# FengHZ/SHOT-VAE

Hardware: AMD Instinct MI355X
Metric: images/sec/step WRN-28-2 SHOT-VAE CIFAR-10 bs512 (higher is better)
Workload: dtype bf16; 1 GPU; SHOT-VAE train step (4 fwd + 2 bwd + SGD) wideresnet-28-2 K=10 ldc=128, B_l=B_u=512 per GPU, synthetic 3x32x32 in HBM, random init; global_batch=1024, parallelism=dp1, schedule=grouped (forwards (1)-(4) as one batched launch sequence, 4 BatchNorm groups), launch=eager, weight gradients on a side stream, collective=none

## Files before the change

include/shotvae_hip.h:

```cpp
#ifndef SHOTVAE_HIP_H
#define SHOTVAE_HIP_H

#include <stdint.h>

#ifdef __cplusplus
extern "C" {
#endif

#define SV_ABI_VERSION 8

enum { SV_F32 = 0, SV_BF16 = 1 };
typedef double sv_acc_t;
enum { SV_OK = 0, SV_E_ARG = -1, SV_E_SHAPE = -2, SV_E_HIP = -3 };
enum { SV_MAX_TAPS = 16, SV_MAX_PHASES = 4 };

typedef struct {
    int32_t ooy, oox;
    int32_t ntap;
    int8_t dy[SV_MAX_TAPS];
    int8_t dx[SV_MAX_TAPS];
    int8_t torig[SV_MAX_TAPS];
    int64_t w_off;
} sv_phase;

// ... 276 lines not shown
int sv_prof_enable(int on);
int sv_prof_tag(int tag);
int sv_prof_nested_tag(int tag);
int sv_prof_nested_tag_kind(int kind, int tag);
int sv_prof_collect(int max_tags, double* ms, int* count);

int sv_debug_wgrad_tile_program(int halo_vectors, int* items, int* waits);

int sv_debug_conv_chunk_program(int* items, int* waits);

enum { SV_OPT_DISABLE_MASK = 0, SV_OPT_WIDE_MIN_BLOCKS = 1, SV_OPT_HALO_ALL = 2, SV_OPT_PERSISTENT_BLOCKS = 3,
       SV_OPT_DETERMINISTIC = 4, SV_OPT_ENABLE_MASK = 5 };
enum { SV_K_CONV3X3 = 1, SV_K_CONV3X3P = 2, SV_K_CONV3X3M = 4, SV_K_CONV3X3W = 8, SV_K_CONV3X3X = 16,
       SV_K_WGRAD3X3 = 32, SV_K_WGRAD3X3W = 64, SV_K_IGEMM_KV2 = 128, SV_K_HALO = 256, SV_K_HALOP = 512, SV_K_HWGRAD = 1024, SV_K_IGEMM_BIG = 2048, SV_K_WGRAD_WIDE = 4096, SV_K_IGEMM_ALIGNED = 8192, SV_K_IGEMM_DMA = 16384, SV_K_WGRAD_INCR = 32768, SV_K_WGRAD3X3M = 65536, SV_K_TCONVR = 131072, SV_K_TCONVR_EX = 262144, SV_K_SCONV = 524288, SV_K_PCONV = 8388608, SV_K_THCONV = 16777216, SV_K_THWGRAD = 67108864, SV_K_S2WGRAD = 134217728,
       SV_K_MAP4 = 268435456,
       SV_K_MAP4_CONV = 536870912   };
int sv_set_option(int key, int value);
int sv_get_option(int key);

int sv_stream_fork(void* from, void* to, int light);
int sv_stream_flag_next(void* stream, uint32_t** flag, uint32_t* value);
int sv_stream_wait_flag(void* stream, const uint32_t* flag, uint32_t value);
int sv_flag_timeouts(void);
int sv_flag_timeouts_reset(void);

int sv_version(void);
const char* sv_last_error(void);

#ifdef __cplusplus
}
#endif
// ... 2 lines not shown
```

shot_vae_amd/_lib.py:

```python
import ctypes as C
import os
import subprocess

HERE = os.path.dirname(os.path.abspath(__file__))
LIB_PATH = os.environ.get("SV_LIB_PATH") or os.path.join(HERE, "libshotvae_hip.so")
CSRC = os.path.join(HERE, "csrc")

SV_F32, SV_BF16 = 0, 1
ABI_VERSION = 8
MAX_TAPS, MAX_PHASES = 16, 4


class SvPhase(C.Structure):
    _fields_ = [("ooy", C.c_int32), ("oox", C.c_int32), ("ntap", C.c_int32),
                ("dy", C.c_int8 * MAX_TAPS), ("dx", C.c_int8 * MAX_TAPS), ("torig", C.c_int8 * MAX_TAPS),
                ("w_off", C.c_int64)]


class SvGeom(C.Structure):
    _fields_ = [("B", C.c_int32), ("Hin", C.c_int32), ("Win", C.c_int32), ("Cin", C.c_int32), ("ldx", C.c_int32),
                ("Hq", C.c_int32), ("Wq", C.c_int32), ("sy", C.c_int32), ("sx", C.c_int32),
                ("Hout", C.c_int32), ("Wout", C.c_int32), ("N", C.c_int32), ("ldo", C.c_int32),
                ("osy", C.c_int32), ("osx", C.c_int32), ("T_orig", C.c_int32), ("nphase", C.c_int32),
                ("phase", SvPhase * MAX_PHASES)]
# ... 151 lines not shown
    "sv_bn_bwd_apply_dropout": [I, I64, I, I, P, P, P, F, C.POINTER(SvBnBranch), I, P, P, I, C.POINTER(SvDropoutArgs), P],
    "sv_dropout_mask": [P, I, C.c_uint32, I64, I, I, P, P],
    "sv_stream_fork": [P, P, I],
    "sv_stream_flag_next": [P, P, P],
    "sv_stream_wait_flag": [P, P, C.c_uint32],
    "sv_flag_timeouts": [],
    "sv_flag_timeouts_reset": [],
    "sv_version": [],
}
OPT_DISABLE_MASK, OPT_WIDE_MIN_BLOCKS, OPT_HALO_ALL, OPT_PERSISTENT_BLOCKS, OPT_DETERMINISTIC, OPT_ENABLE_MASK = 0, 1, 2, 3, 4, 5
(K_CONV3X3, K_CONV3X3P, K_CONV3X3M, K_CONV3X3W, K_CONV3X3X, K_WGRAD3X3, K_WGRAD3X3W, K_IGEMM_KV2, K_HALO, K_HALOP, K_HWGRAD, K_IGEMM_BIG,
 K_WGRAD_WIDE, K_IGEMM_ALIGNED, K_IGEMM_DMA, K_WGRAD_INCR, K_WGRAD3X3M, K_TCONVR, K_TCONVR_EX, K_SCONV) = (1 << i for i in range(20))
K_PCONV, K_THCONV, K_THWGRAD, K_S2WGRAD = 1 << 23, 1 << 24, 1 << 26, 1 << 27
K_MAP4 = 1 << 28
K_MAP4_CONV = 1 << 29
EXPORTS = sorted(list(_PROTOS) + ["sv_last_error"])

_lib = None


class ShotVaeHipError(RuntimeError):
    pass


def build(verbose=False):
    r = subprocess.run(["make", "-C", CSRC, "-j4"], capture_output=True, text=True)
    if verbose or r.returncode != 0:
        print(r.stdout[-4000:])
        print(r.stderr[-4000:])
    if r.returncode != 0:
# ... 87 lines not shown
```

shot_vae_amd/csrc/bwd3x3f.hip:

```cpp
#include "common.h"
#include "epilogue.h"

int sv_bwd3x3_64(const sv_geom* g, const sv_bwd3x3_args* a, hipStream_t s);

namespace {

constexpr int LDF = 48;
constexpr int LDR = 40;
constexpr int CH = 32;
#ifndef SV_BWDF_WREGS
#define SV_BWDF_WREGS 2
#endif
#ifndef SV_BWDF_ABL
#define SV_BWDF_ABL 0
#endif

struct bwdf_params {
    const void* dy;
    const void* dy2;
    const void* dy3;
    void* dy_out;
    const float* dy_scale;
    const float* dy_scale2;
    const float* dy_shift;
// ... 18 lines not shown
    int fold_replicas;
};
struct bwdf_g { bwdf_params g[SV_MAX_GROUPS]; };

__device__ __forceinline__ bf16x8 ftr(const bf16* S, int pix_elem_q, int col0, int lane) {
    typedef __attribute__((address_space(3))) s16x4 lds_v4;
    const bf16* a0 = S + pix_elem_q + col0 + 4 * (lane & 3);
    const s16x4 lo = __builtin_amdgcn_ds_read_tr16_b64_v4i16((lds_v4*)(a0));
    const s16x4 hi = __builtin_amdgcn_ds_read_tr16_b64_v4i16((lds_v4*)(a0 + 4 * LDF));
    union { s16x4 s[2]; bf16x8 b; } u;
    u.s[0] = lo;
    u.s[1] = hi;
    return u.b;
}

template <int NS, int MODE>
struct bwdf_stage {
    bf16x8 gv[NS];
    bf16x8 yv[MODE >= 1 ? NS : 1];
    bf16x8 rv[MODE == 2 ? NS : 1];
    bf16x8 xv;
};

template <int WLOG, int MODE>
__global__ __launch_bounds__(512) void bwd3x3f_kernel(const sv_geom g, const bwdf_g PG) {
    const bwdf_params& p = PG.g[blockIdx.y];
    typedef bf16x8 V;
    typedef bf16x4 Q;
    constexpr int WREGS = WLOG == 5 ? SV_BWDF_WREGS : (MODE == 0 ? 1 : 0);
    constexpr int FRAGS = WLOG == 5 ? 1 : 2;
    constexpr bool GFIRST = MODE >= 1;
    constexpr int WLROWS = (2 - WREGS) * 16 * 9;
    constexpr int W = 1 << WLOG, TR = 128 / W, WP = W + 2;
    constexpr int HH = (TR < W) ? TR : W, SEG = TR / HH, LROWS = TR + SEG + 1, HP = LROWS * WP;
    constexpr int HV = LROWS * W * 4;
    static_assert(HV > 512 && HV <= 768, "slots: vectors 0..511 on the weight-gradient waves (two each), 512.. on the others (one each)");
    constexpr int SDY = HP * LDF, SAC = 128 * LDF, SXR = 128 * LDR, STG = SDY + SAC + SXR;
    static_assert((SDY * 2) % 16 == 0 && (SAC * 2) % 16 == 0 && (STG * 2) % 16 == 0, "16-byte aligned LDS images");

    extern __shared__ __attribute__((aligned(16))) char smem[];
    bf16* const st0 = reinterpret_cast<bf16*>(smem);
    double* const ssum = reinterpret_cast<double*>(st0 + 2 * STG);
    float* const cf = reinterpret_cast<float*>(ssum + 2 * CH);
    bf16* const wl = reinterpret_cast<bf16*>(cf + 8 * CH);

    const int tid = threadIdx.x, lane = tid & 63;
    const int wave = __builtin_amdgcn_readfirstlane(tid >> 6);
// ... 9 lines not shown
    const char* __restrict__ X = reinterpret_cast<const char*>(p.x);
    bf16* __restrict__ O = reinterpret_cast<bf16*>(p.out);
    float slope = p.x_slope;
    asm volatile("v_mov_b32 %0, %0" : "+v"(slope));

    if (MODE >= 1 && p.fold_bsums) {
        sv_bn_bwd_affine_block512<CH>(p.fold_bsums, p.fold_replicas, p.fold_inv_count, p.fold_gamma, p.fold_mean, p.fold_rstd,
                                      p.fold_dgamma, p.fold_dbeta, blockIdx.x == 0, reinterpret_cast<double*>(smem), cf);
    }
    if (tid < CH) {
        if (MODE >= 1 && !p.fold_bsums) {
            cf[tid] = p.dy_scale[tid];
            cf[CH + tid] = p.dy_scale2[tid];
            cf[2 * CH + tid] = p.dy_shift[tid];
        }
        cf[3 * CH + tid] = p.x_scale[tid];
        cf[4 * CH + tid] = p.x_shift[tid];
        cf[5 * CH + tid] = p.x_mean[tid];
        cf[6 * CH + tid] = p.x_rstd[tid];
    }
    if (tid < 2 * CH) ssum[tid] = 0.0;
    for (int idx = tid; idx < 2 * LROWS * 2 * 4; idx += 512) {
        const int vv = idx & 3, side = (idx >> 2) & 1, row = (idx >> 3) % LROWS, stg = (idx >> 3) / LROWS;
        bf16x8 z;
#pragma unroll
        for (int j = 0; j < 8; ++j) z[j] = (bf16)0.f;
        *reinterpret_cast<bf16x8*>(st0 + stg * STG + (row * WP + side * (WP - 1)) * LDF + 8 * vv) = z;
    }

    const int v = tid & 3;
    int hlds[2];
    uint32_t hoff[2];
#pragma unroll
    for (int i = 0; i < 2; ++i) {
        const int idx = wave >= 4 ? (tid - 256) + 256 * i : (i == 0 ? 512 + tid : HV);
        const int pix = min(idx, HV - 1) >> 2;
        const int lr = pix >> WLOG, xx = pix & (W - 1);
        const int seg = lr / (HH + 1), off = lr - seg * (HH + 1);
        int kind = 1, rel = lr - 1 - seg;
        if (off == 0) {
            if (SEG == 1) { kind = seg == 0 ? 2 : 3; rel = seg == 0 ? -1 : TR; }
            else kind = 0;
        }
        hoff[i] = (uint32_t)(((rel + 1) * W + xx) * CH + 8 * v) * 2u;
        hlds[i] = idx < HV ? (((lr * WP + xx + 1) * LDF + 8 * v) | kind) : -1;
    }
    const uint32_t hsafe = (uint32_t)(W * CH + 8 * v) * 2u;
    const int cp = tid >> 2;
    const uint32_t coff = (uint32_t)(cp * CH + 8 * v) * 2u;

    auto load_stage = [&](auto& S, int tile) __attribute__((always_inline)) {
        constexpr int NS = sizeof(S.gv) / sizeof(V);
        const int gr0 = tile * TR;
        const bool top_ok = (gr0 & (H - 1)) != 0, bot_ok = ((gr0 + TR) & (H - 1)) != 0;
        const int64_t hb = ((int64_t)gr0 - 1) * W * CH * 2;
#pragma unroll
        for (int i = 0; i < NS; ++i) {
            const int kind = hlds[i] & 3;
            const bool ok = hlds[i] >= 0 && (kind == 1 || (kind == 2 && top_ok) || (kind == 3 && bot_ok));
            const uint32_t o = ok ? hoff[i] : hsafe;
            S.gv[i] = *reinterpret_cast<const V*>(DY + hb + o);
            if constexpr (MODE >= 1) S.yv[i] = *reinterpret_cast<const V*>(DY2 + hb + o);
            if constexpr (MODE == 2) S.rv[i] = *reinterpret_cast<const V*>(DY3 + hb + o);
        }
        S.xv = *reinterpret_cast<const V*>(X + (int64_t)gr0 * W * CH * 2 + coff);
    };
    V zero;
#pragma unroll
    for (int j = 0; j < 8; ++j) zero[j] = (bf16)0.f;
    auto store_stage = [&](auto& S, int tile, int stage) __attribute__((always_inline)) {
        constexpr int NS = sizeof(S.gv) / sizeof(V);
        bf16* sb = st0 + stage * STG;
        const int gr0 = tile * TR;
        const bool top_ok = (gr0 & (H - 1)) != 0, bot_ok = ((gr0 + TR) & (H - 1)) != 0;
        const int64_t hb = ((int64_t)gr0 - 1) * W * CH * 2;
#pragma unroll
        for (int i = 0; i < NS; ++i) {
            const int kind = hlds[i] & 3;
            const bool ok = kind == 1 || (kind == 2 && top_ok) || (kind == 3 && bot_ok);
            V o = S.gv[i];
// ... 5 lines not shown
                    const f32x4 cc = *reinterpret_cast<const f32x4*>(cf + 2 * CH + 8 * v + 4 * h);
#pragma unroll
                    for (int j = 0; j < 4; ++j) {
                        float t = to_f(S.gv[i][4 * h + j]) * ca[j] + (to_f(S.yv[MODE >= 1 ? i : 0][4 * h + j]) * cb[j] + cc[j]);
                        if constexpr (MODE == 2) t += to_f(S.rv[MODE == 2 ? i : 0][4 * h + j]);
                        o[4 * h + j] = (bf16)t;
                    }
                }
                if constexpr (MODE == 2) {
                    if (hlds[i] >= 0 && kind == 1) *reinterpret_cast<V*>(DYO + hb + hoff[i]) = o;
                }
            }
            if (!ok) o = zero;
            if (hlds[i] >= 0) *reinterpret_cast<V*>(sb + (hlds[i] & ~7)) = o;
        }
        const f32x4 s0 = *reinterpret_cast<const f32x4*>(cf + 3 * CH + 8 * v), s1 = *reinterpret_cast<const f32x4*>(cf + 3 * CH + 8 * v + 4);
        const f32x4 t0 = *reinterpret_cast<const f32x4*>(cf + 4 * CH + 8 * v), t1 = *reinterpret_cast<const f32x4*>(cf + 4 * CH + 8 * v + 4);
        *reinterpret_cast<V*>(sb + SDY + cp * LDF + 8 * v) = bn_act8(S.xv, s0, s1, t0, t1, slope);
        *reinterpret_cast<V*>(sb + SDY + SAC + cp * LDR + 8 * v) = S.xv;
    };

    const int dwave = wave & 3;
    int hbase[2], prow[2], pcol[2];
#pragma unroll
    for (int ms = 0; ms < 2; ++ms) {
        const int pp = 32 * dwave + 16 * ms + fr;
        prow[ms] = pp >> WLOG;
        pcol[ms] = pp & (W - 1);
        hbase[ms] = ((prow[ms] + 1 + prow[ms] / HH) * WP + pcol[ms] + 1) * LDF + 8 * fq;
    }
    V wr[9][WREGS > 0 ? WREGS : 1];
    float s1[2][4], s2[2][4];
#pragma unroll
    for (int i = 0; i < 2; ++i)
#pragma unroll
        for (int r = 0; r < 4; ++r) s1[i][r] = s2[i][r] = 0.f;
    {
        const bf16* Wp = reinterpret_cast<const bf16*>(p.w) + P.w_off;
        if (wave < 4) {
#pragma unroll
            for (int t = 0; t < 9; ++t)
#pragma unroll
                for (int i = 0; i < WREGS; ++i) wr[t][i] = *reinterpret_cast<const V*>(Wp + ((16 * i + fr) * 9 + t) * CH + 8 * fq);
        }
        for (int idx = tid; idx < WLROWS * 4; idx += 512)
            *reinterpret_cast<V*>(wl + (idx >> 2) * LDF + 8 * (idx & 3)) =
                *reinterpret_cast<const V*>(Wp + (WREGS * 16 * 9 + (idx >> 2)) * CH + 8 * (idx & 3));
    }
    auto compute_d = [&](int tile, int stage) __attribute__((always_inline)) {
        const bf16* dyh = st0 + stage * STG;
        const bf16* xr = dyh + SDY + SAC;
        f32x4 acc[2][2];
#pragma unroll
        for (int i = 0; i < 2; ++i)
#pragma unroll
            for (int j = 0; j < 2; ++j) acc[i][j] = f32x4{0.f, 0.f, 0.f, 0.f};
#pragma unroll
        for (int t = 0; t < 9; ++t) {
            const int sh = ((1 - t / 3) * WP + (1 - t % 3)) * LDF;
            const V af0 = *reinterpret_cast<const V*>(dyh + hbase[0] + sh);
            const V af1 = *reinterpret_cast<const V*>(dyh + hbase[1] + sh);
#pragma unroll
            for (int i = 0; i < 2; ++i) {
                const V wf = i < WREGS ? wr[t][i < WREGS ? i : 0] : *reinterpret_cast<const V*>(wl + (((i - WREGS) * 16 + fr) * 9 + t) * LDF + 8 * fq);
                mma32(acc[i][0], wf, af0);
                mma32(acc[i][1], wf, af1);
            }
        }
        const int gr0 = tile * TR;
        if (SV_BWDF_ABL & 16) {
#pragma unroll
            for (int i = 0; i < 2; ++i)
#pragma unroll
                for (int ms = 0; ms < 2; ++ms) s1[i][ms] += acc[i][ms][0] + acc[i][ms][1] + acc[i][ms][2] + acc[i][ms][3];
            return;
        }
#pragma unroll
        for (int i = 0; i < 2; ++i) {
            const int c = 16 * i + 4 * fq;
            const f32x4 esc = *reinterpret_cast<const f32x4*>(cf + 3 * CH + c), esh = *reinterpret_cast<const f32x4*>(cf + 4 * CH + c);
            const f32x4 emu = *reinterpret_cast<const f32x4*>(cf + 5 * CH + c), ers = *reinterpret_cast<const f32x4*>(cf + 6 * CH + c);
#pragma unroll
            for (int ms = 0; ms < 2; ++ms) {
                const Q xq = *reinterpret_cast<const Q*>(xr + (32 * dwave + 16 * ms + fr) * LDR + c);
                f32x4 vv = acc[i][ms];
                Q o;
#pragma unroll
                for (int r = 0; r < 4; ++r) {
                    const float xf = to_f(xq[r]);
                    const float gv = vv[r] * act_grad(xf * esc[r] + esh[r], slope);
                    s1[i][r] += gv;
                    s2[i][r] += gv * ((xf - emu[r]) * ers[r]);
                    o[r] = (bf16)gv;
                }
                *reinterpret_cast<Q*>(O + ((int64_t)(gr0 + prow[ms]) * W + pcol[ms]) * CH + c) = o;
            }
        }
    };

    const int wi = (wave >> 1) & 1, wj = wave & 1;
    f32x4 dacc[9];
#pragma unroll
    for (int t = 0; t < 9; ++t) dacc[t] = f32x4{0.f, 0.f, 0.f, 0.f};
    auto compute_g = [&](int stage) __attribute__((always_inline)) {
        const bf16* dyh = st0 + stage * STG;
        const bf16* ac = dyh + SDY;
        auto frag_b = [&](int kc) __attribute__((always_inline)) {
            const int pq = 32 * kc + 8 * fq + (fr >> 2);
            return ftr(ac, pq * LDF, 16 * wj, lane);
        };
        auto frag_a = [&](int kc, int t) __attribute__((always_inline)) {
            const int pq = 32 * kc + 8 * fq + (fr >> 2);
            const int jrow = pq >> WLOG, xcol = pq & (W - 1);
            const int hb = ((jrow + 1 + jrow / HH) * WP + xcol + 1) * LDF;
            return ftr(dyh, hb + ((1 - t / 3) * WP + (1 - t % 3)) * LDF, 16 * wi, lane);
        };
        if constexpr (FRAGS == 1) {
#pragma unroll
            for (int kc = 0; kc < 4; ++kc) {
                const bf16x8 fb = frag_b(kc);
                bf16x8 fa[9];
#pragma unroll
                for (int t = 0; t < 9; ++t) fa[t] = frag_a(kc, t);
#pragma unroll
                for (int t = 0; t < 9; ++t) dacc[t] = __builtin_amdgcn_mfma_f32_16x16x32_bf16(fa[t], fb, dacc[t], 0, 0, 0);
            }
        } else {
#pragma unroll
            for (int kc = 0; kc < 4; ++kc) {
                const bf16x8 fb = frag_b(kc);
                bf16x8 fa[5];
#pragma unroll
                for (int t = 0; t < 5; ++t) fa[t] = frag_a(kc, t);
#pragma unroll
                for (int t = 0; t < 5; ++t) dacc[t] = __builtin_amdgcn_mfma_f32_16x16x32_bf16(fa[t], fb, dacc[t], 0, 0, 0);
#pragma unroll
                for (int t = 5; t < 9; ++t) fa[t - 5] = frag_a(kc, t);
#pragma unroll
                for (int t = 5; t < 9; ++t) dacc[t] = __builtin_amdgcn_mfma_f32_16x16x32_bf16(fa[t - 5], fb, dacc[t], 0, 0, 0);
            }
        }
    };

    auto tile_barrier = [&]() __attribute__((always_inline)) { asm volatile("s_waitcnt lgkmcnt(0)\n\ts_barrier" ::: "memory"); };
// ... 11 lines not shown
        load_stage(SB, min(t_begin + tstep, t_last));
        __syncthreads();
        store_stage(SA, t_begin, 0);
        load_stage(SA, min(t_begin + 2 * tstep, t_last));
        __syncthreads();
        int tile = t_begin;
        for (int k = 0; k + 1 < n_tiles; k += 2, tile += 2 * tstep) {
            iter(tile, 0, SB);
            iter(tile + tstep, 1, SA);
        }
        if (n_tiles & 1) {
            if (!(SV_BWDF_ABL & 2)) compute_d(tile, 0);
            tile_barrier();
        }
#pragma unroll
        for (int i = 0; i < 2; ++i)
#pragma unroll
            for (int r = 0; r < 4; ++r) {
                s1[i][r] = row16_sum(s1[i][r]);
                s2[i][r] = row16_sum(s2[i][r]);
            }
        if (fr == 0) {
#pragma unroll
            for (int i = 0; i < 2; ++i)
#pragma unroll
                for (int r = 0; r < 4; ++r) {
                    atomicAdd(&ssum[16 * i + 4 * fq + r], (double)s1[i][r]);
                    atomicAdd(&ssum[CH + 16 * i + 4 * fq + r], (double)s2[i][r]);
                }
        }
    } else {
        bwdf_stage<2, MODE> SA, SB;
        auto iter = [&](int tile, int stage, bwdf_stage<2, MODE>& S) __attribute__((always_inline)) {
            if (!GFIRST && !(SV_BWDF_ABL & 1)) compute_g(stage);
            if (!(SV_BWDF_ABL & 8)) store_stage(S, min(tile + tstep, t_last), stage ^ 1);
            if (!(SV_BWDF_ABL & 4)) load_stage(S, min(tile + 3 * tstep, t_last));
            if (GFIRST && !(SV_BWDF_ABL & 1)) compute_g(stage);
            tile_barrier();
        };
        load_stage(SA, t_begin);
        load_stage(SB, min(t_begin + tstep, t_last));
        __syncthreads();
        store_stage(SA, t_begin, 0);
        load_stage(SA, min(t_begin + 2 * tstep, t_last));
        __syncthreads();
        int tile = t_begin;
        for (int k = 0; k + 1 < n_tiles; k += 2, tile += 2 * tstep) {
            iter(tile, 0, SB);
            iter(tile + tstep, 1, SA);
        }
        if (n_tiles & 1) {
            if (!(SV_BWDF_ABL & 1)) compute_g(0);
            tile_barrier();
        }
        float* dst = p.ws + ((int64_t)blockIdx.y * gridDim.x + blockIdx.x) * (9 * CH * CH);
#pragma unroll
        for (int t = 0; t < 9; ++t) {
#pragma unroll
            for (int r = 0; r < 4; ++r) dst[((16 * wi + 4 * fq + r) * 9 + t) * CH + 16 * wj + fr] = dacc[t][r];
        }
    }
    __syncthreads();
    if (tid < 2 * CH) {
        double* dst = p.bsums + (size_t)(blockIdx.x & (p.replicas - 1)) * 2 * CH;
        atomicAdd(dst + tid, ssum[tid]);
    }
}

template <int WLOG, int MODE>
int launch(const sv_geom* g, const bwdf_g& PG, int grid, int groups, hipStream_t s) {
    constexpr int W = 1 << WLOG, TR = 128 / W, WP = W + 2;
    constexpr int HH = (TR < W) ? TR : W, LROWS = TR + TR / HH + 1, HP = LROWS * WP;
    constexpr int WREGS = WLOG == 5 ? SV_BWDF_WREGS : (MODE == 0 ? 1 : 0);
    constexpr size_t lds = (size_t)2 * (HP * LDF + 128 * LDF + 128 * LDR) * 2 + 2 * CH * 8 + 8 * CH * 4 + (size_t)(2 - WREGS) * 16 * 9 * LDF * 2;
    static bool optin = false;
    if (const int rc = sv_lds_optin(optin, (int)lds, "bwd3x3f", &bwd3x3f_kernel<WLOG, MODE>)) return rc;
    sv_prof_begin(s);
    hipLaunchKernelGGL((bwd3x3f_kernel<WLOG, MODE>), dim3(grid, groups), dim3(512), lds, s, *g, PG);
    sv_prof_end(s);
    return sv_check_launch("sv_bwd3x3");
}

}

extern "C" int sv_bwd3x3(const sv_geom* g, int dtype, const sv_bwd3x3_args* a, void* stream) {
    SV_REQUIRE(g && a, SV_E_ARG, "sv_bwd3x3: null argument");
    SV_REQUIRE(dtype == SV_BF16, SV_E_ARG, "sv_bwd3x3: bf16 only (dtype=%d)", dtype);
    SV_REQUIRE(a->dy && a->x && a->w && a->out && a->dw && a->ws && a->bsums, SV_E_ARG, "sv_bwd3x3: null tensor");
    SV_REQUIRE(a->x_scale && a->x_shift && a->x_mean && a->x_rstd, SV_E_ARG, "sv_bwd3x3: the BatchNorm vectors of x are required");
    SV_REQUIRE(a->x_slope >= 0.f && a->x_slope <= 1.f, SV_E_ARG, "sv_bwd3x3: slope %g outside [0, 1]", (double)a->x_slope);
    SV_REQUIRE(!a->dy2 || a->fold_bsums || (a->dy_scale && a->dy_scale2 && a->dy_shift), SV_E_ARG,
               "sv_bwd3x3: the two-tensor dy operand needs dy_scale, dy_scale2 and dy_shift (or the fold_* sums)");
    SV_REQUIRE(!a->fold_bsums || (a->dy2 && a->fold_gamma && a->fold_mean && a->fold_rstd && a->fold_replicas >= 1 && a->fold_count > 0.f),
               SV_E_ARG, "sv_bwd3x3: incomplete BatchNorm-backward fold (fold_* need dy2, gamma, mean, rstd, replicas >= 1, count > 0)");
    SV_REQUIRE((a->dy3 != nullptr) == (a->dy_out != nullptr) && (!a->dy3 || a->dy2), SV_E_ARG,
               "sv_bwd3x3: the residual form needs dy2 (+ coefficients), dy3 AND dy_out");
    const int groups = sv_ngroups(a->groups);
    SV_REQUIRE(groups <= SV_MAX_GROUPS, SV_E_ARG, "sv_bwd3x3: groups=%d", groups);
    SV_REQUIRE(a->replicas >= 1 && (a->replicas & (a->replicas - 1)) == 0, SV_E_ARG, "sv_bwd3x3: replicas=%d", a->replicas);
    const bool shape_ok = g->nphase == 1 && g->phase[0].ntap == 9 && g->T_orig == 9 && g->sy == 1 && g->sx == 1 && g->osy == 1 &&
                          g->osx == 1 && g->Hq == g->Hin && g->Wq == g->Win && g->Hout == g->Hin && g->Wout == g->Win &&
                          g->Hin == g->Win && g->Cin == g->N && g->ldx == g->Cin && g->ldo == g->N && g->phase[0].ooy == 0 &&
                          g->phase[0].oox == 0 &&
                          ((g->Cin == CH && (g->Win == 8 || g->Win == 16 || g->Win == 32)) || (g->Cin == 64 && g->Win == 16));
    SV_REQUIRE(shape_ok, SV_E_SHAPE, "sv_bwd3x3: stride-1 3x3 layers with 32 -> 32 channels on 8 / 16 / 32-pixel maps or 64 -> 64 channels on 16-pixel maps only");
    for (int t = 0; t < 9; ++t)
        SV_REQUIRE(g->phase[0].dy[t] == 1 - t / 3 && g->phase[0].dx[t] == 1 - t % 3 && g->phase[0].torig[t] == t, SV_E_SHAPE,
                   "sv_bwd3x3: tap %d is not the data-gradient tap of geometry.convT_like(k = 3, stride = 1, pad = 1)", t);
    const int TR = g->Cin == 64 ? 4 : 128 / g->Win;
    SV_REQUIRE((g->B * g->Hin) % TR == 0, SV_E_SHAPE, "sv_bwd3x3: B * H = %d is not a multiple of the %d-row tile", g->B * g->Hin, TR);
    SV_REQUIRE(!sv_deterministic() && !sv_det_stats(), SV_E_ARG, "sv_bwd3x3: not available in deterministic mode (use the pair)");
    if (g->Cin == 64) return sv_bwd3x3_64(g, a, (hipStream_t)stream);
    const int nT = g->B * g->Hin / TR;
    int budget = a->block_budget > 0 ? a->block_budget : 256;
    int grid = budget / groups;
    if (grid > nT) grid = nT;
    if (grid < 1) grid = 1;
    const int64_t slab = 9 * CH * CH;
    SV_REQUIRE(a->ws_elems >= (int64_t)grid * groups * slab, SV_E_ARG, "sv_bwd3x3: workspace of %lld floats, %lld needed",
               (long long)a->ws_elems, (long long)((int64_t)grid * groups * slab));
    hipStream_t s = (hipStream_t)stream;
    bwdf_g PG;
    const int64_t ts = (int64_t)g->B * g->Hin * g->Win * CH * 2;
    for (int64_t grp = 0; grp < SV_MAX_GROUPS; ++grp) {
        const int64_t q = grp < groups ? grp : 0;
        bwdf_params& r = PG.g[grp];
        r.dy = reinterpret_cast<const char*>(a->dy) + q * ts;
        r.dy2 = a->dy2 ? reinterpret_cast<const char*>(a->dy2) + q * ts : nullptr;
        r.dy3 = a->dy3 ? reinterpret_cast<const char*>(a->dy3) + q * ts : nullptr;
        r.dy_out = a->dy_out ? reinterpret_cast<char*>(a->dy_out) + q * ts : nullptr;
        const bool fold = a->dy2 && a->fold_bsums;
        r.dy_scale = a->dy2 && !fold ? a->dy_scale + q * CH : nullptr;
        r.dy_scale2 = a->dy2 && !fold ? a->dy_scale2 + q * CH : nullptr;
        r.dy_shift = a->dy2 && !fold ? a->dy_shift + q * CH : nullptr;
        r.fold_bsums = fold ? a->fold_bsums + q * (int64_t)a->fold_replicas * 2 * CH : nullptr;
        r.fold_gamma = a->fold_gamma;
        r.fold_mean = fold ? a->fold_mean + q * CH : nullptr;
        r.fold_rstd = fold ? a->fold_rstd + q * CH : nullptr;
        r.fold_dgamma = a->fold_dgamma;
        r.fold_dbeta = a->fold_dbeta;
        r.fold_inv_count = fold ? 1.f / a->fold_count : 0.f;
        r.fold_replicas = a->fold_replicas;
        r.x = reinterpret_cast<const char*>(a->x) + q * ts;
        r.x_scale = a->x_scale + q * CH;
        r.x_shift = a->x_shift + q * CH;
        r.x_mean = a->x_mean + q * CH;
        r.x_rstd = a->x_rstd + q * CH;
        r.x_slope = a->x_slope;
        r.w = a->w;
        r.out = reinterpret_cast<char*>(a->out) + q * ts;
        r.bsums = a->bsums + q * (int64_t)a->replicas * 2 * CH;
        r.replicas = a->replicas;
        r.ws = a->ws;
    }
    int rc;
    const int mode = a->dy3 ? 2 : a->dy2 ? 1 : 0;
    switch (g->Win * 4 + mode) {
        case 32 * 4 + 0: rc = launch<5, 0>(g, PG, grid, groups, s); break;
        case 32 * 4 + 1: rc = launch<5, 1>(g, PG, grid, groups, s); break;
        case 32 * 4 + 2: rc = launch<5, 2>(g, PG, grid, groups, s); break;
        case 16 * 4 + 0: rc = launch<4, 0>(g, PG, grid, groups, s); break;
        case 16 * 4 + 1: rc = launch<4, 1>(g, PG, grid, groups, s); break;
        case 16 * 4 + 2: rc = launch<4, 2>(g, PG, grid, groups, s); break;
        case 8 * 4 + 0: rc = launch<3, 0>(g, PG, grid, groups, s); break;
        case 8 * 4 + 1: rc = launch<3, 1>(g, PG, grid, groups, s); break;
        default: rc = launch<3, 2>(g, PG, grid, groups, s); break;
    }
    if (rc != SV_OK) return rc;
    sv_slab_reduce(a->ws, grid * groups, slab, a->dw, s);
    return sv_check_launch("sv_bwd3x3(slab reduce)");
}
```

shot_vae_amd/engine.py:

```python
import ctypes as C
import os
import math
import re

import torch

from . import _lib as L
from . import geometry as G
_GEOM = G

LEAKY_SLOPE = 0.01
BN_EPS = 1e-5
BN_MOMENTUM = 0.1
CPAD = 16


def _align(n, a=64):
    return (n + a - 1) // a * a


def _pad16(c):
    return (c + CPAD - 1) // CPAD * CPAD


# ... 426 lines not shown
            pool = self._ws = {}
        key = (torch.cuda.current_stream().cuda_stream, self.param.device)
        ws = pool.get(key)
        if ws is None:
            ws = pool[key] = torch.empty(self._ws_elems, dtype=torch.float32, device=self.param.device)
        return ws

    wgrad_side_stream = True
    sparse_shortcut_grad = True
    compact_shortcut_grad = True
    materialize_decoder_act = True
    materialize_max_hin = 4
    light_fork = True
    fork_every = 1
    fused_bwd = 2
    fold_bn_bwd = True
    fused_channels = (32, 64)
    fused_blocks = 248
    flag_fork = True
    _fused_since_fork = False
    event_fork_after_fused = True
    _start_signal = None
    _pending_wgrads = ()
    fold_bn = True

    def _side(self):
        pool = getattr(self, "_side_streams", None)
        if pool is None:
            pool = self._side_streams = {}
        cur = torch.cuda.current_stream()
        s = pool.get(cur.cuda_stream)
        if s is None:
            s = pool[cur.cuda_stream] = torch.cuda.Stream()
# ... 67 lines not shown

    def _wgrad(self, g, x, pro, dy, dw_ptr, tag=None, groups=1, budget=0):
        if tag:
            self._tag(tag, g, wgrad=True, groups=groups)
        a = L.SvWgradArgs()
        a.x, a.dy, a.dw = x.data_ptr(), dy.data_ptr(), dw_ptr
        if pro is not None:
            a.pro_scale, a.pro_shift, a.pro_slope = pro[0], pro[1], pro[2]
        a.splits, a.use_tr, a.ws, a.ws_elems = 0, self.use_tr, self._wg_ws().data_ptr(), self._ws_elems
        a.groups, a.block_budget = groups, budget
        L.call("sv_wgrad_ex", C.byref(g), self.code, C.byref(a), self._stream())

    def _bwd3x3(self, cv, B, dy, lin2, x, bn_ptrs, slope, out, bsums, replicas, tag, groups, budget=0, res=None):
        g = cv.geom_dgrad(B)
        if tag:
            n = groups * g.B * g.Hin * g.Win * g.Cin
            es = self.packs.element_size()
            if self.prof_tags is not None:
                L.lib().sv_prof_tag(self.prof_tags.setdefault(tag, len(self.prof_tags)))
            self._cost(tag, es * n * (3 + (lin2 is not None) + 2 * (res is not None)) + 4 * 9 * g.Cin * g.N, 2 * 2.0 * n * 9 * g.N)
        a = L.SvBwd3x3Args()
        a.dy, a.x, a.out = dy.data_ptr(), x.data_ptr(), out.data_ptr()
        if lin2 is not None and len(lin2) == 2:
            a.dy2 = lin2[0].data_ptr()
            (a.fold_bsums, a.fold_replicas, a.fold_count, a.fold_gamma, a.fold_mean, a.fold_rstd, a.fold_dgamma, a.fold_dbeta) = lin2[1]
        elif lin2 is not None:
            a.dy2, a.dy_scale, a.dy_scale2, a.dy_shift = lin2[0].data_ptr(), lin2[1], lin2[2], lin2[3]
        if res is not None:
            a.dy3, a.dy_out = res[0].data_ptr(), res[1].data_ptr()
        a.x_scale, a.x_shift, a.x_mean, a.x_rstd = bn_ptrs
        a.x_slope = slope
        a.w = self.packs.data_ptr() + self.packs.element_size() * cv.dgrad_off
        a.bsums, a.replicas, a.groups = bsums, replicas, groups
        a.dw = self.grad.data_ptr() + 4 * cv.master_off
        a.ws, a.ws_elems, a.block_budget = self._wg_ws().data_ptr(), self._ws_elems, budget or self.fused_blocks
        self._fused_since_fork = True
        L.call("sv_bwd3x3", C.byref(g), self.code, C.byref(a), self._stream())

    def _dropout_fwd(self, c1, unit, keys, stats, replicas, groups):
        c = c1.shape[-1]
        tag = "fwd:dropout_%d" % c
        if self.prof_tags is not None:
            L.lib().sv_prof_tag(self.prof_tags.setdefault(tag, len(self.prof_tags)))
        self._cost(tag, 2 * c1.numel() * c1.element_size())
        a = L.dropout_args(keys.data_ptr(), unit, self.drop_rate)
        L.call("sv_dropout_fwd", self.code, _vp(c1.data_ptr()), c1.numel() // c // groups, c, c, C.byref(a), _vp(c1.data_ptr()),
               _vp(stats), replicas, groups, self._stream())

    def _bn_layout(self, G):
# ... 433 lines not shown
                del lin2n, g1n, Dres
            elif fb >= 3:
                self._bwd3x3(un["conv2"], B, D, None, c1, bnp(un["bn2"]), un["bn2"].slope, g2, bs_off[un["bn2"].index],
                             bs_rep[un["bn2"].index], "bwd:conv3x3_%dx%d_s1" % (c, c), G)
            else:
                self._wgrad_async(un["conv2"].geom_fwd(B), c1, pro2, D, gbase + 4 * un["conv2"].master_off,
                                  tag="wgrad:conv3x3_%dx%d_s1" % (c, c), groups=G, budget=pair,
                                  then=lambda: self._igemm(un["conv2"].geom_dgrad(B), D, pk + es * un["conv2"].dgrad_off, g2,
                                                           ex=ex_of(un["bn2"], c1), tag="dgrad:conv3x3_%dx%d_s1" % (c, c),
                                                           groups=G, budget=pair))
            pair1 = pair if same else (min(pair, self.pair_blocks_strided) if self.prof_tags is None else 0)
            cnt = tin.numel() // tin.shape[-1] // G
            g1 = torch.empty_like(tin)
            tag1 = "conv3x3_%dx%d_s%d" % (un["cin"], c, un["stride"])
            drop_unit = i if f.drop_keys is not None else None
            if fb >= 1 and same and drop_unit is None:
                if self.fold_bn_bwd:
                    lin21 = (c1, bn_fold(un["bn2"], cnt2))
                else:
                    coef, sg, sx, sh = bn_affine(un["bn2"], cnt2)
                    lin21 = (c1, sg, sx, sh)
                self._bwd3x3(un["conv1"], B, g2, lin21, tin, bnp(un["bn1"]), un["bn1"].slope, g1,
                             bs_off[un["bn1"].index], bs_rep[un["bn1"].index], "bwd:" + tag1 + "+bn", G)
                del lin21
                dc1 = None
            else:
                dc1 = bn_apply(c1, [(g2, un["bn2"])], None, cnt2, drop_unit=drop_unit)
                self._wgrad_async(un["conv1"].geom_fwd(B), tin, pro1, dc1, gbase + 4 * un["conv1"].master_off,
                                  tag="wgrad:" + tag1, groups=G, budget=pair1,
                                  then=lambda: self._igemm(un["conv1"].geom_dgrad(B), dc1, pk + es * un["conv1"].dgrad_off, g1,
                                                           ex=ex_of(un["bn1"], tin), tag="dgrad:" + tag1, groups=G, budget=pair1))
# ... 36 lines not shown
```

Baseline: 166,000 images/s.

## Add thin 16->32 channel form of the fused 3x3 backward kernel

Extends the fused backward 3x3 kernel (data gradient + BN backward + weight gradient) with a thin variant for 16-input, 32-output layers on 32x32 maps. The two wave halves reduce their weight-gradient partials in LDS before writing to the workspace. The engine gains a fused_thin switch to route the first block-group conv1 through this kernel, but it defaults to False. The default fused block budget also changes from a fixed 248 to the device CU count minus 8.

```diff
diff --git a/include/shotvae_hip.h b/include/shotvae_hip.h
--- a/include/shotvae_hip.h
+++ b/include/shotvae_hip.h
@@ -314,7 +314,8 @@
 enum { SV_K_CONV3X3 = 1, SV_K_CONV3X3P = 2, SV_K_CONV3X3M = 4, SV_K_CONV3X3W = 8, SV_K_CONV3X3X = 16,
        SV_K_WGRAD3X3 = 32, SV_K_WGRAD3X3W = 64, SV_K_IGEMM_KV2 = 128, SV_K_HALO = 256, SV_K_HALOP = 512, SV_K_HWGRAD = 1024, SV_K_IGEMM_BIG = 2048, SV_K_WGRAD_WIDE = 4096, SV_K_IGEMM_ALIGNED = 8192, SV_K_IGEMM_DMA = 16384, SV_K_WGRAD_INCR = 32768, SV_K_WGRAD3X3M = 65536, SV_K_TCONVR = 131072, SV_K_TCONVR_EX = 262144, SV_K_SCONV = 524288, SV_K_PCONV = 8388608, SV_K_THCONV = 16777216, SV_K_THWGRAD = 67108864, SV_K_S2WGRAD = 134217728,
        SV_K_MAP4 = 268435456,
-       SV_K_MAP4_CONV = 536870912   };
+       SV_K_MAP4_CONV = 536870912,
+       SV_K_BWD_THIN = 1073741824   };
 int sv_set_option(int key, int value);
 int sv_get_option(int key);
 
diff --git a/shot_vae_amd/_lib.py b/shot_vae_amd/_lib.py
--- a/shot_vae_amd/_lib.py
+++ b/shot_vae_amd/_lib.py
@@ -189,6 +189,7 @@
 K_PCONV, K_THCONV, K_THWGRAD, K_S2WGRAD = 1 << 23, 1 << 24, 1 << 26, 1 << 27
 K_MAP4 = 1 << 28
 K_MAP4_CONV = 1 << 29
+K_BWD_THIN = 1 << 30
 EXPORTS = sorted(list(_PROTOS) + ["sv_last_error"])
 
 _lib = None
diff --git a/shot_vae_amd/csrc/bwd3x3f.hip b/shot_vae_amd/csrc/bwd3x3f.hip
--- a/shot_vae_amd/csrc/bwd3x3f.hip
+++ b/shot_vae_amd/csrc/bwd3x3f.hip
@@ -1,3 +1,5 @@
+#include <type_traits>
+
 #include "common.h"
 #include "epilogue.h"
 
@@ -56,23 +58,27 @@
     return u.b;
 }
 
-template <int NS, int MODE>
+template <int NS, int MODE, bool HASX = true>
 struct bwdf_stage {
+    static constexpr bool has_x = HASX;
     bf16x8 gv[NS];
     bf16x8 yv[MODE >= 1 ? NS : 1];
     bf16x8 rv[MODE == 2 ? NS : 1];
     bf16x8 xv;
 };
 
-template <int WLOG, int MODE>
+template <int WLOG, int MODE, int XC>
 __global__ __launch_bounds__(512) void bwd3x3f_kernel(const sv_geom g, const bwdf_g PG) {
     const bwdf_params& p = PG.g[blockIdx.y];
     typedef bf16x8 V;
     typedef bf16x4 Q;
-    constexpr int WREGS = WLOG == 5 ? SV_BWDF_WREGS : (MODE == 0 ? 1 : 0);
+    static_assert(XC == CH || (XC == 16 && WLOG == 5 && MODE <= 1), "the thin form: 32 x 32 maps, no residual form");
+    constexpr int NT = XC / 16;
+    constexpr bool THIN = XC != CH;
+    constexpr int WREGS = THIN ? 1 : WLOG == 5 ? SV_BWDF_WREGS : (MODE == 0 ? 1 : 0);
     constexpr int FRAGS = WLOG == 5 ? 1 : 2;
     constexpr bool GFIRST = MODE >= 1;
-    constexpr int WLROWS = (2 - WREGS) * 16 * 9;
+    constexpr int WLROWS = (NT - WREGS) * 16 * 9;
     constexpr int W = 1 << WLOG, TR = 128 / W, WP = W + 2;
     constexpr int HH = (TR < W) ? TR : W, SEG = TR / HH, LROWS = TR + SEG + 1, HP = LROWS * WP;
     constexpr int HV = LROWS * W * 4;
@@ -112,12 +118,14 @@
             cf[CH + tid] = p.dy_scale2[tid];
             cf[2 * CH + tid] = p.dy_shift[tid];
         }
+    }
+    if (tid < XC) {
         cf[3 * CH + tid] = p.x_scale[tid];
         cf[4 * CH + tid] = p.x_shift[tid];
         cf[5 * CH + tid] = p.x_mean[tid];
         cf[6 * CH + tid] = p.x_rstd[tid];
     }
-    if (tid < 2 * CH) ssum[tid] = 0.0;
+    if (tid < 2 * XC) ssum[tid] = 0.0;
     for (int idx = tid; idx < 2 * LROWS * 2 * 4; idx += 512) {
         const int vv = idx & 3, side = (idx >> 2) & 1, row = (idx >> 3) % LROWS, stg = (idx >> 3) / LROWS;
         bf16x8 z;
@@ -144,8 +152,8 @@
         hlds[i] = idx < HV ? (((lr * WP + xx + 1) * LDF + 8 * v) | kind) : -1;
     }
     const uint32_t hsafe = (uint32_t)(W * CH + 8 * v) * 2u;
-    const int cp = tid >> 2;
-    const uint32_t coff = (uint32_t)(cp * CH + 8 * v) * 2u;
+    const int cp = THIN ? (tid >> 1) & 127 : tid >> 2, xg = THIN ? tid & 1 : v;
+    const uint32_t coff = (uint32_t)(cp * XC + 8 * xg) * 2u;
 
     auto load_stage = [&](auto& S, int tile) __attribute__((always_inline)) {
         constexpr int NS = sizeof(S.gv) / sizeof(V);
@@ -161,7 +169,7 @@
             if constexpr (MODE >= 1) S.yv[i] = *reinterpret_cast<const V*>(DY2 + hb + o);
             if constexpr (MODE == 2) S.rv[i] = *reinterpret_cast<const V*>(DY3 + hb + o);
         }
-        S.xv = *reinterpret_cast<const V*>(X + (int64_t)gr0 * W * CH * 2 + coff);
+        if constexpr (std::remove_reference_t<decltype(S)>::has_x) S.xv = *reinterpret_cast<const V*>(X + (int64_t)gr0 * W * XC * 2 + coff);
     };
     V zero;
 #pragma unroll
@@ -197,10 +205,12 @@
             if (!ok) o = zero;
             if (hlds[i] >= 0) *reinterpret_cast<V*>(sb + (hlds[i] & ~7)) = o;
         }
-        const f32x4 s0 = *reinterpret_cast<const f32x4*>(cf + 3 * CH + 8 * v), s1 = *reinterpret_cast<const f32x4*>(cf + 3 * CH + 8 * v + 4);
-        const f32x4 t0 = *reinterpret_cast<const f32x4*>(cf + 4 * CH + 8 * v), t1 = *reinterpret_cast<const f32x4*>(cf + 4 * CH + 8 * v + 4);
-        *reinterpret_cast<V*>(sb + SDY + cp * LDF + 8 * v) = bn_act8(S.xv, s0, s1, t0, t1, slope);
-        *reinterpret_cast<V*>(sb + SDY + SAC + cp * LDR + 8 * v) = S.xv;
+        if constexpr (std::remove_reference_t<decltype(S)>::has_x) {
+            const f32x4 s0 = *reinterpret_cast<const f32x4*>(cf + 3 * CH + 8 * xg), s1 = *reinterpret_cast<const f32x4*>(cf + 3 * CH + 8 * xg + 4);
+            const f32x4 t0 = *reinterpret_cast<const f32x4*>(cf + 4 * CH + 8 * xg), t1 = *reinterpret_cast<const f32x4*>(cf + 4 * CH + 8 * xg + 4);
+            *reinterpret_cast<V*>(sb + SDY + cp * LDF + 8 * xg) = bn_act8(S.xv, s0, s1, t0, t1, slope);
+            *reinterpret_cast<V*>(sb + SDY + SAC + cp * LDR + 8 * xg) = S.xv;
+        }
     };
 
     const int dwave = wave & 3;
@@ -213,9 +223,9 @@
         hbase[ms] = ((prow[ms] + 1 + prow[ms] / HH) * WP + pcol[ms] + 1) * LDF + 8 * fq;
     }
     V wr[9][WREGS > 0 ? WREGS : 1];
-    float s1[2][4], s2[2][4];
-#pragma unroll
-    for (int i = 0; i < 2; ++i)
+    float s1[NT][4], s2[NT][4];
+#pragma unroll
+    for (int i = 0; i < NT; ++i)
 #pragma unroll
         for (int r = 0; r < 4; ++r) s1[i][r] = s2[i][r] = 0.f;
     {
@@ -233,9 +243,9 @@
     auto compute_d = [&](int tile, int stage) __attribute__((always_inline)) {
         const bf16* dyh = st0 + stage * STG;
         const bf16* xr = dyh + SDY + SAC;
-        f32x4 acc[2][2];
-#pragma unroll
-        for (int i = 0; i < 2; ++i)
+        f32x4 acc[NT][2];
+#pragma unroll
+        for (int i = 0; i < NT; ++i)
 #pragma unroll
             for (int j = 0; j < 2; ++j) acc[i][j] = f32x4{0.f, 0.f, 0.f, 0.f};
 #pragma unroll
@@ -244,7 +254,7 @@
             const V af0 = *reinterpret_cast<const V*>(dyh + hbase[0] + sh);
             const V af1 = *reinterpret_cast<const V*>(dyh + hbase[1] + sh);
 #pragma unroll
-            for (int i = 0; i < 2; ++i) {
+            for (int i = 0; i < NT; ++i) {
                 const V wf = i < WREGS ? wr[t][i < WREGS ? i : 0] : *reinterpret_cast<const V*>(wl + (((i - WREGS) * 16 + fr) * 9 + t) * LDF + 8 * fq);
                 mma32(acc[i][0], wf, af0);
                 mma32(acc[i][1], wf, af1);
@@ -253,13 +263,13 @@
         const int gr0 = tile * TR;
         if (SV_BWDF_ABL & 16) {
 #pragma unroll
-            for (int i = 0; i < 2; ++i)
+            for (int i = 0; i < NT; ++i)
 #pragma unroll
                 for (int ms = 0; ms < 2; ++ms) s1[i][ms] += acc[i][ms][0] + acc[i][ms][1] + acc[i][ms][2] + acc[i][ms][3];
             return;
         }
 #pragma unroll
-        for (int i = 0; i < 2; ++i) {
+        for (int i = 0; i < NT; ++i) {
             const int c = 16 * i + 4 * fq;
             const f32x4 esc = *reinterpret_cast<const f32x4*>(cf + 3 * CH + c), esh = *reinterpret_cast<const f32x4*>(cf + 4 * CH + c);
             const f32x4 emu = *reinterpret_cast<const f32x4*>(cf + 5 * CH + c), ers = *reinterpret_cast<const f32x4*>(cf + 6 * CH + c);
@@ -276,12 +286,13 @@
                     s2[i][r] += gv * ((xf - emu[r]) * ers[r]);
                     o[r] = (bf16)gv;
                 }
-                *reinterpret_cast<Q*>(O + ((int64_t)(gr0 + prow[ms]) * W + pcol[ms]) * CH + c) = o;
+                *reinterpret_cast<Q*>(O + ((int64_t)(gr0 + prow[ms]) * W + pcol[ms]) * XC + c) = o;
             }
         }
     };
 
-    const int wi = (wave >> 1) & 1, wj = wave & 1;
+    const int wi = (wave >> 1) & 1, wj = THIN ? 0 : wave & 1, wh = THIN ? wave & 1 : 0;
+    constexpr int NKC = THIN ? 2 : 4;
     f32x4 dacc[9];
 #pragma unroll
     for (int t = 0; t < 9; ++t) dacc[t] = f32x4{0.f, 0.f, 0.f, 0.f};
@@ -289,18 +300,18 @@
         const bf16* dyh = st0 + stage * STG;
         const bf16* ac = dyh + SDY;
         auto frag_b = [&](int kc) __attribute__((always_inline)) {
-            const int pq = 32 * kc + 8 * fq + (fr >> 2);
+            const int pq = 32 * (kc + NKC * wh) + 8 * fq + (fr >> 2);
             return ftr(ac, pq * LDF, 16 * wj, lane);
         };
         auto frag_a = [&](int kc, int t) __attribute__((always_inline)) {
-            const int pq = 32 * kc + 8 * fq + (fr >> 2);
+            const int pq = 32 * (kc + NKC * wh) + 8 * fq + (fr >> 2);
             const int jrow = pq >> WLOG, xcol = pq & (W - 1);
             const int hb = ((jrow + 1 + jrow / HH) * WP + xcol + 1) * LDF;
             return ftr(dyh, hb + ((1 - t / 3) * WP + (1 - t % 3)) * LDF, 16 * wi, lane);
         };
         if constexpr (FRAGS == 1) {
 #pragma unroll
-            for (int kc = 0; kc < 4; ++kc) {
+            for (int kc = 0; kc < NKC; ++kc) {
                 const bf16x8 fb = frag_b(kc);
                 bf16x8 fa[9];
 #pragma unroll
@@ -310,7 +321,7 @@
             }
         } else {
 #pragma unroll
-            for (int kc = 0; kc < 4; ++kc) {
+            for (int kc = 0; kc < NKC; ++kc) {
                 const bf16x8 fb = frag_b(kc);
                 bf16x8 fa[5];
 #pragma unroll
@@ -352,7 +363,7 @@
             tile_barrier();
         }
 #pragma unroll
-        for (int i = 0; i < 2; ++i)
+        for (int i = 0; i < NT; ++i)
 #pragma unroll
             for (int r = 0; r < 4; ++r) {
                 s1[i][r] = row16_sum(s1[i][r]);
@@ -360,16 +371,16 @@
             }
         if (fr == 0) {
 #pragma unroll
-            for (int i = 0; i < 2; ++i)
+            for (int i = 0; i < NT; ++i)
 #pragma unroll
                 for (int r = 0; r < 4; ++r) {
                     atomicAdd(&ssum[16 * i + 4 * fq + r], (double)s1[i][r]);
-                    atomicAdd(&ssum[CH + 16 * i + 4 * fq + r], (double)s2[i][r]);
+                    atomicAdd(&ssum[XC + 16 * i + 4 * fq + r], (double)s2[i][r]);
                 }
         }
     } else {
-        bwdf_stage<2, MODE> SA, SB;
-        auto iter = [&](int tile, int stage, bwdf_stage<2, MODE>& S) __attribute__((always_inline)) {
+        bwdf_stage<2, MODE, !THIN> SA, SB;
+        auto iter = [&](int tile, int stage, bwdf_stage<2, MODE, !THIN>& S) __attribute__((always_inline)) {
             if (!GFIRST && !(SV_BWDF_ABL & 1)) compute_g(stage);
             if (!(SV_BWDF_ABL & 8)) store_stage(S, min(tile + tstep, t_last), stage ^ 1);
             if (!(SV_BWDF_ABL & 4)) load_stage(S, min(tile + 3 * tstep, t_last));
@@ -391,30 +402,37 @@
             if (!(SV_BWDF_ABL & 1)) compute_g(0);
             tile_barrier();
         }
-        float* dst = p.ws + ((int64_t)blockIdx.y * gridDim.x + blockIdx.x) * (9 * CH * CH);
+        float* dst = THIN ? reinterpret_cast<float*>(smem) + wh * (9 * CH * XC)
+                          : p.ws + ((int64_t)blockIdx.y * gridDim.x + blockIdx.x) * (9 * CH * XC);
 #pragma unroll
         for (int t = 0; t < 9; ++t) {
 #pragma unroll
-            for (int r = 0; r < 4; ++r) dst[((16 * wi + 4 * fq + r) * 9 + t) * CH + 16 * wj + fr] = dacc[t][r];
+            for (int r = 0; r < 4; ++r) dst[((16 * wi + 4 * fq + r) * 9 + t) * XC + 16 * wj + fr] = dacc[t][r];
         }
     }
     __syncthreads();
-    if (tid < 2 * CH) {
-        double* dst = p.bsums + (size_t)(blockIdx.x & (p.replicas - 1)) * 2 * CH;
+    if constexpr (THIN) {
+        static_assert(2 * 9 * CH * XC * 4 <= 2 * STG * 2, "both halves of the slab fit the stage area");
+        const float* red = reinterpret_cast<const float*>(smem);
+        float* dst = p.ws + ((int64_t)blockIdx.y * gridDim.x + blockIdx.x) * (9 * CH * XC);
+        for (int idx = tid; idx < 9 * CH * XC; idx += 512) dst[idx] = red[idx] + red[9 * CH * XC + idx];
+    }
+    if (tid < 2 * XC) {
+        double* dst = p.bsums + (size_t)(blockIdx.x & (p.replicas - 1)) * 2 * XC;
         atomicAdd(dst + tid, ssum[tid]);
     }
 }
 
-template <int WLOG, int MODE>
+template <int WLOG, int MODE, int XC = CH>
 int launch(const sv_geom* g, const bwdf_g& PG, int grid, int groups, hipStream_t s) {
     constexpr int W = 1 << WLOG, TR = 128 / W, WP = W + 2;
     constexpr int HH = (TR < W) ? TR : W, LROWS = TR + TR / HH + 1, HP = LROWS * WP;
-    constexpr int WREGS = WLOG == 5 ? SV_BWDF_WREGS : (MODE == 0 ? 1 : 0);
-    constexpr size_t lds = (size_t)2 * (HP * LDF + 128 * LDF + 128 * LDR) * 2 + 2 * CH * 8 + 8 * CH * 4 + (size_t)(2 - WREGS) * 16 * 9 * LDF * 2;
+    constexpr int WREGS = XC != CH ? 1 : WLOG == 5 ? SV_BWDF_WREGS : (MODE == 0 ? 1 : 0);
+    constexpr size_t lds = (size_t)2 * (HP * LDF + 128 * LDF + 128 * LDR) * 2 + 2 * CH * 8 + 8 * CH * 4 + (size_t)(XC / 16 - WREGS) * 16 * 9 * LDF * 2;
     static bool optin = false;
-    if (const int rc = sv_lds_optin(optin, (int)lds, "bwd3x3f", &bwd3x3f_kernel<WLOG, MODE>)) return rc;
+    if (const int rc = sv_lds_optin(optin, (int)lds, "bwd3x3f", &bwd3x3f_kernel<WLOG, MODE, XC>)) return rc;
     sv_prof_begin(s);
-    hipLaunchKernelGGL((bwd3x3f_kernel<WLOG, MODE>), dim3(grid, groups), dim3(512), lds, s, *g, PG);
+    hipLaunchKernelGGL((bwd3x3f_kernel<WLOG, MODE, XC>), dim3(grid, groups), dim3(512), lds, s, *g, PG);
     sv_prof_end(s);
     return sv_check_launch("sv_bwd3x3");
 }
@@ -438,10 +456,12 @@
     SV_REQUIRE(a->replicas >= 1 && (a->replicas & (a->replicas - 1)) == 0, SV_E_ARG, "sv_bwd3x3: replicas=%d", a->replicas);
     const bool shape_ok = g->nphase == 1 && g->phase[0].ntap == 9 && g->T_orig == 9 && g->sy == 1 && g->sx == 1 && g->osy == 1 &&
                           g->osx == 1 && g->Hq == g->Hin && g->Wq == g->Win && g->Hout == g->Hin && g->Wout == g->Win &&
-                          g->Hin == g->Win && g->Cin == g->N && g->ldx == g->Cin && g->ldo == g->N && g->phase[0].ooy == 0 &&
-                          g->phase[0].oox == 0 &&
-                          ((g->Cin == CH && (g->Win == 8 || g->Win == 16 || g->Win == 32)) || (g->Cin == 64 && g->Win == 16));
-    SV_REQUIRE(shape_ok, SV_E_SHAPE, "sv_bwd3x3: stride-1 3x3 layers with 32 -> 32 channels on 8 / 16 / 32-pixel maps or 64 -> 64 channels on 16-pixel maps only");
+                          g->Hin == g->Win && g->ldx == g->Cin && g->ldo == g->N && g->phase[0].ooy == 0 && g->phase[0].oox == 0 &&
+                          ((g->Cin == CH && g->N == CH && (g->Win == 8 || g->Win == 16 || g->Win == 32)) ||
+                           (g->Cin == CH && g->N == 16 && g->Win == 32) || (g->Cin == 64 && g->N == 64 && g->Win == 16));
+    SV_REQUIRE(shape_ok, SV_E_SHAPE, "sv_bwd3x3: stride-1 3x3 layers with 32 -> 32 channels on 8 / 16 / 32-pixel maps, 16 -> 32 channels on 32-pixel maps or 64 -> 64 channels on 16-pixel maps only");
+    const int XC = g->N;
+    SV_REQUIRE(XC == g->Cin || !a->dy3, SV_E_ARG, "sv_bwd3x3: no residual form for a 16 -> 32 channel layer (it has no identity skip)");
     for (int t = 0; t < 9; ++t)
         SV_REQUIRE(g->phase[0].dy[t] == 1 - t / 3 && g->phase[0].dx[t] == 1 - t % 3 && g->phase[0].torig[t] == t, SV_E_SHAPE,
                    "sv_bwd3x3: tap %d is not the data-gradient tap of geometry.convT_like(k = 3, stride = 1, pad = 1)", t);
@@ -454,12 +474,13 @@
     int grid = budget / groups;
     if (grid > nT) grid = nT;
     if (grid < 1) grid = 1;
-    const int64_t slab = 9 * CH * CH;
+    const int64_t slab = 9 * CH * XC;
     SV_REQUIRE(a->ws_elems >= (int64_t)grid * groups * slab, SV_E_ARG, "sv_bwd3x3: workspace of %lld floats, %lld needed",
                (long long)a->ws_elems, (long long)((int64_t)grid * groups * slab));
     hipStream_t s = (hipStream_t)stream;
     bwdf_g PG;
     const int64_t ts = (int64_t)g->B * g->Hin * g->Win * CH * 2;
+    const int64_t tx = (int64_t)g->B * g->Hin * g->Win * XC * 2;
     for (int64_t grp = 0; grp < SV_MAX_GROUPS; ++grp) {
         const int64_t q = grp < groups ? grp : 0;
         bwdf_params& r = PG.g[grp];
@@ -479,21 +500,22 @@
         r.fold_dbeta = a->fold_dbeta;
         r.fold_inv_count = fold ? 1.f / a->fold_count : 0.f;
         r.fold_replicas = a->fold_replicas;
-        r.x = reinterpret_cast<const char*>(a->x) + q * ts;
-        r.x_scale = a->x_scale + q * CH;
-        r.x_shift = a->x_shift + q * CH;
-        r.x_mean = a->x_mean + q * CH;
-        r.x_rstd = a->x_rstd + q * CH;
+        r.x = reinterpret_cast<const char*>(a->x) + q * tx;
+        r.x_scale = a->x_scale + q * XC;
+        r.x_shift = a->x_shift + q * XC;
+        r.x_mean = a->x_mean + q * XC;
+        r.x_rstd = a->x_rstd + q * XC;
         r.x_slope = a->x_slope;
         r.w = a->w;
-        r.out = reinterpret_cast<char*>(a->out) + q * ts;
-        r.bsums = a->bsums + q * (int64_t)a->replicas * 2 * CH;
+        r.out = reinterpret_cast<char*>(a->out) + q * tx;
+        r.bsums = a->bsums + q * (int64_t)a->replicas * 2 * XC;
         r.replicas = a->replicas;
         r.ws = a->ws;
     }
     int rc;
     const int mode = a->dy3 ? 2 : a->dy2 ? 1 : 0;
-    switch (g->Win * 4 + mode) {
+    if (XC != CH) rc = mode == 0 ? launch<5, 0, 16>(g, PG, grid, groups, s) : launch<5, 1, 16>(g, PG, grid, groups, s);
+    else switch (g->Win * 4 + mode) {
         case 32 * 4 + 0: rc = launch<5, 0>(g, PG, grid, groups, s); break;
         case 32 * 4 + 1: rc = launch<5, 1>(g, PG, grid, groups, s); break;
         case 32 * 4 + 2: rc = launch<5, 2>(g, PG, grid, groups, s); break;
diff --git a/shot_vae_amd/engine.py b/shot_vae_amd/engine.py
--- a/shot_vae_amd/engine.py
+++ b/shot_vae_amd/engine.py
@@ -464,9 +464,10 @@
     light_fork = True
     fork_every = 1
     fused_bwd = 2
+    fused_thin = False
     fold_bn_bwd = True
     fused_channels = (32, 64)
-    fused_blocks = 248
+    fused_blocks = 0
     flag_fork = True
     _fused_since_fork = False
     event_fork_after_fused = True
@@ -564,11 +565,12 @@
     def _bwd3x3(self, cv, B, dy, lin2, x, bn_ptrs, slope, out, bsums, replicas, tag, groups, budget=0, res=None):
         g = cv.geom_dgrad(B)
         if tag:
-            n = groups * g.B * g.Hin * g.Win * g.Cin
+            npix = groups * g.B * g.Hin * g.Win
             es = self.packs.element_size()
             if self.prof_tags is not None:
                 L.lib().sv_prof_tag(self.prof_tags.setdefault(tag, len(self.prof_tags)))
-            self._cost(tag, es * n * (3 + (lin2 is not None) + 2 * (res is not None)) + 4 * 9 * g.Cin * g.N, 2 * 2.0 * n * 9 * g.N)
+            self._cost(tag, es * npix * (g.Cin * (1 + (lin2 is not None) + 2 * (res is not None)) + 2 * g.N) + 4 * 9 * g.Cin * g.N,
+                       2 * 2.0 * npix * 9 * g.Cin * g.N)
         a = L.SvBwd3x3Args()
         a.dy, a.x, a.out = dy.data_ptr(), x.data_ptr(), out.data_ptr()
         if lin2 is not None and len(lin2) == 2:
@@ -583,6 +585,8 @@
         a.w = self.packs.data_ptr() + self.packs.element_size() * cv.dgrad_off
         a.bsums, a.replicas, a.groups = bsums, replicas, groups
         a.dw = self.grad.data_ptr() + 4 * cv.master_off
+        if not budget and not self.fused_blocks:
+            self.fused_blocks = max(8, torch.cuda.get_device_properties(self.param.device).multi_processor_count - 8)
         a.ws, a.ws_elems, a.block_budget = self._wg_ws().data_ptr(), self._ws_elems, budget or self.fused_blocks
         self._fused_since_fork = True
         L.call("sv_bwd3x3", C.byref(g), self.code, C.byref(a), self._stream())
@@ -1046,7 +1050,9 @@
             g1 = torch.empty_like(tin)
             tag1 = "conv3x3_%dx%d_s%d" % (un["cin"], c, un["stride"])
             drop_unit = i if f.drop_keys is not None else None
-            if fb >= 1 and same and drop_unit is None:
+            thin = (fb >= 1 and self.fused_thin and un["cin"] == 16 and c == 32 and un["stride"] == 1 and hmap == 32 and
+                    (B * 32) % 4 == 0 and not (L.lib().sv_get_option(L.OPT_DISABLE_MASK) & L.K_BWD_THIN))
+            if fb >= 1 and (same or thin) and drop_unit is None:
                 if self.fold_bn_bwd:
                     lin21 = (c1, bn_fold(un["bn2"], cnt2))
                 else:
```

New measurement: 165,900 images/s. No clear change (-0.1%).
